# chkda/pytorch-distributed-tutorials

Hardware: AMD Instinct MI355X
Metric: images/sec (whole node) ResNet-50 bf16 at 1/2/4/8 MI355X (higher is better)
Workload: dtype bf16; 1 GPU; model=resnet50, global_batch=256, image_size=224, parallelism=dp1, impl=native, backend=nccl, wire_dtype=fp32, comm_backend=auto, cudnn_benchmark=False, graph=False, deterministic=False, force_comm=False, plan_world=1

## Files before the change

csrc/kernels/bn_act.hip:

```cpp
#include "common.h"
#include "fp8_util.h"
#include "igemm_common.h"
#include "kernels.h"
#include "pool_quad.h"

#include <algorithm>
#include <cstdlib>
#include <mutex>
#include <numeric>
#include <stdexcept>
#include <unordered_map>

namespace pdt {

__device__ __forceinline__ void load8(const float* p, float (&v)[8]) {
  float4 a = *reinterpret_cast<const float4*>(p);
  float4 b = *reinterpret_cast<const float4*>(p + 4);
  v[0] = a.x; v[1] = a.y; v[2] = a.z; v[3] = a.w; v[4] = b.x; v[5] = b.y; v[6] = b.z; v[7] = b.w;
}

#ifndef PDT_FIN_CH
#define PDT_FIN_CH 32
#endif
constexpr int FIN_CH = PDT_FIN_CH;
// ... 25 lines not shown
  return b < 0 ? -1 : b * kTileCounters;
}

int bn_counter_bank(hipStream_t st) {
  const int off = counter_bank(st);
  return off < 0 ? -1 : off / kTileCounters;
}

static bool bn_lastblock() {
  static int v = -1;
  if (v < 0) {
    const char* e = getenv("PDT_BN_LASTBLOCK");
    v = (e && e[0] == '0') ? 0 : 1;
  }
  return v == 1;
}

__device__ __forceinline__ void st_wt(float* p, float v) {
  __hip_atomic_store(p, v, __ATOMIC_RELAXED, __HIP_MEMORY_SCOPE_AGENT);
}
__device__ __forceinline__ float ld_wt(const float* p) {
  return __hip_atomic_load(const_cast<float*>(p), __ATOMIC_RELAXED, __HIP_MEMORY_SCOPE_AGENT);
}
__device__ __forceinline__ bool last_block_of_tile(int tile, unsigned int nblocks) {
  __shared__ int s_last;
  asm volatile("s_waitcnt vmcnt(0)" ::: "memory");
  __syncthreads();
  if (threadIdx.x == 0) {
    const unsigned int prev = __hip_atomic_fetch_add(&g_tile_counters[tile], 1u, __ATOMIC_RELAXED,
                                                     __HIP_MEMORY_SCOPE_AGENT);
    const bool last = prev == nblocks - 1;
    if (last) __hip_atomic_store(&g_tile_counters[tile], 0u, __ATOMIC_RELAXED, __HIP_MEMORY_SCOPE_AGENT);
    s_last = last ? 1 : 0;
  }
  __syncthreads();
  return s_last != 0;
}

__global__ void __launch_bounds__(256) bn_finalize_kernel(const float* __restrict__ part, int ngroups,
                                                          int grows, int M, int K,
                                                          float* __restrict__ ws,
                                                          float* __restrict__ rm,
                                                          float* __restrict__ rv,
                                                          const float* __restrict__ gamma,
                                                          const float* __restrict__ beta,
                                                          float momentum, float eps,
                                                          float* __restrict__ out, int mode,
                                                          int nparts, int cbase, int gpb) {
  __shared__ float sS[FIN_ROWS][FIN_CH + 1], sA[FIN_ROWS][FIN_CH + 1], sB[FIN_ROWS][FIN_CH + 1];
  const int tx = threadIdx.x & (FIN_CH - 1), ty = threadIdx.x / FIN_CH;
  const int k = blockIdx.x * FIN_CH + tx;
  const int g0 = blockIdx.y * gpb;
  const int g1 = min(ngroups, g0 + gpb);
  float S = 0.f, A = 0.f, B = 0.f;
  if (mode != 2) {
  if (k < K) {
#pragma unroll 8
    for (int g = g0 + ty; g < g1; g += FIN_ROWS) {
      const float cnt = (float)min(grows, M - g * grows);
      const float sg = part[((int64_t)g * 2 + 0) * K + k];
      const float qg = part[((int64_t)g * 2 + 1) * K + k];
      S += sg;
      A += qg;
      B = fmaf(sg, sg / cnt, B);
    }
  }
  sS[ty][tx] = S; sA[ty][tx] = A; sB[ty][tx] = B;
  __syncthreads();
  const bool direct = mode == 0 && gridDim.y == 1;
  if (ty == 0 && k < K) {
    for (int r = 1; r < FIN_ROWS; ++r) { S += sS[r][tx]; A += sA[r][tx]; B += sB[r][tx]; }
    if (!direct) {
      float* o = ws + ((int64_t)blockIdx.y * 3) * K;
      st_wt(o + k, S); st_wt(o + K + k, A); st_wt(o + 2 * K + k, B);
    }
  }
  if (mode == 1) return;
  if (direct) {
    if (ty != 0 || k >= K) return;
  } else if (!last_block_of_tile(cbase + blockIdx.x, gridDim.y)) {
    return;
  }
  }
  const bool direct = mode == 0 && gridDim.y == 1;
  const int P = mode == 2 ? nparts : gridDim.y;
  if (!direct) {
  S = 0.f; A = 0.f; B = 0.f;
  if (k < K) {
#pragma unroll 8
    for (int p = ty; p < P; p += FIN_ROWS) {
      const float* o = ws + ((int64_t)p * 3) * K;
      S += ld_wt(o + k); A += ld_wt(o + K + k); B += ld_wt(o + 2 * K + k);
    }
  }
  sS[ty][tx] = S; sA[ty][tx] = A; sB[ty][tx] = B;
  __syncthreads();
  if (ty != 0 || k >= K) return;
  for (int r = 1; r < FIN_ROWS; ++r) { S += sS[r][tx]; A += sA[r][tx]; B += sB[r][tx]; }
  }
  const float mu = S / (float)M;
  const float m2 = fmaxf(A + B - S * mu, 0.f);
  const float var = m2 / (float)M;
  const float invstd = rsqrtf(var + eps);
  if (rm != nullptr) {
    const float unb = M > 1 ? m2 / (float)(M - 1) : var;
    rm[k] = (1.f - momentum) * rm[k] + momentum * mu;
    rv[k] = (1.f - momentum) * rv[k] + momentum * unb;
  }
  const float sc = gamma[k] * invstd;
  out[k] = mu;
  out[K + k] = invstd;
  out[2 * K + k] = sc;
  out[3 * K + k] = beta[k] - mu * sc;
}

int bn_finalize_partitions(int ngroups) { return ceil_div(ngroups, fin_gpb(ngroups)); }

void launch_bn_finalize(const float* part, int ngroups, int grows, int M, int K, float* rm, float* rv,
                        const float* gamma, const float* beta, float momentum, float eps,
                        float* out, hipStream_t st) {
  const int gpb = fin_gpb(ngroups);
  int P = ceil_div(ngroups, gpb);
  float* ws = out + 4 * (int64_t)K;
  if (ceil_div(K, FIN_CH) > kTileCounters / 2) throw std::runtime_error("bn_finalize: too many channels");
  const int bank = (bn_lastblock() && P > 1) ? counter_bank(st) : 0;
  if (bn_lastblock() && bank >= 0) {
    hipLaunchKernelGGL(bn_finalize_kernel, dim3(ceil_div(K, FIN_CH), P), dim3(256), 0, st, part,
                       ngroups, grows, M, K, ws, rm, rv, gamma, beta, momentum, eps, out, 0, P,
                       bank, gpb);
  } else {
    hipLaunchKernelGGL(bn_finalize_kernel, dim3(ceil_div(K, FIN_CH), P), dim3(256), 0, st, part,
                       ngroups, grows, M, K, ws, rm, rv, gamma, beta, momentum, eps, out, 1, P, 0, gpb);
    hipLaunchKernelGGL(bn_finalize_kernel, dim3(ceil_div(K, FIN_CH), 1), dim3(256), 0, st, part,
                       ngroups, grows, M, K, ws, rm, rv, gamma, beta, momentum, eps, out, 2, P, 0, gpb);
  }
}

__global__ void __launch_bounds__(256) bn_finalize_sums_kernel(double* __restrict__ acc, int M, int K,
                                                               float* __restrict__ rm, float* __restrict__ rv,
                                                               const float* __restrict__ gamma,
                                                               const float* __restrict__ beta, float momentum,
                                                               float eps, float* __restrict__ out) {
  const int k = blockIdx.x * blockDim.x + threadIdx.x;
  if (k >= K) return;
  double s[kStatSlots], q[kStatSlots];
#pragma unroll
  for (int x = 0; x < kStatSlots; ++x) {
    s[x] = acc[(size_t)x * 2 * K + k];
    q[x] = acc[(size_t)x * 2 * K + K + k];
  }
  const float g = gamma[k], bt = beta[k];
  const float rm0 = rm != nullptr ? rm[k] : 0.f, rv0 = rm != nullptr ? rv[k] : 0.f;
  double S = 0.0, Q = 0.0;
#pragma unroll
  for (int x = 0; x < kStatSlots; ++x) {
    S += s[x];
    Q += q[x];
    acc[(size_t)x * 2 * K + k] = 0.0;
    acc[(size_t)x * 2 * K + K + k] = 0.0;
  }
  const double Md = (double)M;
  const double mu = S / Md;
  const double var = fmax(Q / Md - mu * mu, 0.0);
  const float invstd = rsqrtf((float)var + eps);
  if (rm != nullptr) {
    const float unb = M > 1 ? (float)(var * Md / (Md - 1.0)) : (float)var;
    rm[k] = (1.f - momentum) * rm0 + momentum * (float)mu;
    rv[k] = (1.f - momentum) * rv0 + momentum * unb;
  }
  const float sc = g * invstd;
  out[k] = (float)mu;
  out[K + k] = invstd;
  out[2 * K + k] = sc;
  out[3 * K + k] = bt - (float)mu * sc;
}

void launch_bn_finalize_sums(const BnFwdFuse& bn, int M, int K, hipStream_t st) {
  hipLaunchKernelGGL(bn_finalize_sums_kernel, dim3(ceil_div(K, 256)), dim3(256), 0, st, bn.acc, M, K, bn.rm,
                     bn.rv, bn.gamma, bn.beta, bn.momentum, bn.eps, bn.out);
}

struct FoldCoef {
  const float* stats;
  const float* gamma;
  const float* sums;
  int K;
  float invM;
  __device__ __forceinline__ void ab(int k, float& a, float& b) const {
    const float is = stats[K + k], mu = stats[k];
    const float k1 = gamma[k] * is;
    const float k2 = sums[K + k] * is * is * invM;
    a = -k1 * k2;
    b = -k1 * (sums[k] * invM - mu * k2);
  }
};

constexpr int kFoldMaxK = 2048;
constexpr int kCsumSlots = 128, kCsumBlocks = 4096;
typedef __bf16 fold_v8bf __attribute__((ext_vector_type(8)));

__global__ void __launch_bounds__(256) bn_fold_coef_kernel(FoldCoef cf, float* __restrict__ coef) {
  __builtin_amdgcn_s_setprio(3);
  const int k = blockIdx.x * 256 + threadIdx.x;
  if (k < cf.K) cf.ab(k, coef[k], coef[cf.K + k]);
}

__global__ void __launch_bounds__(256) bn_fold_weights_kernel(const uint16_t* __restrict__ wt, FoldCoef cf,
                                                              const float* __restrict__ coef, int C, int nG,
                                                              uint16_t* __restrict__ wfold,
                                                              float* __restrict__ bias,
                                                              float* __restrict__ part) {
  __builtin_amdgcn_s_setprio(3);
  const int K = cf.K, t = threadIdx.x;
  const int KC = K + C;
  const int bid = blockIdx.x;
  if (bid >= nG) {
    const int64_t e = ((int64_t)(bid - nG) * 256 + t) * 8;
    if (e >= (int64_t)C * K) return;
    const int c = (int)(e / K), k = (int)(e - (int64_t)c * K);
    f8 v = unpack8(*reinterpret_cast<const uint4*>(wt + e));
    float g8[8], i8[8];
    load8(cf.gamma + k, g8);
    load8(cf.stats + K + k, i8);
#pragma unroll
    for (int q = 0; q < 8; ++q) v.v[q] *= g8[q] * i8[q];
    *reinterpret_cast<uint4*>(wfold + (size_t)c * KC + k) = pack8(v);
    return;
  }
  const int nt = C / 32;
  const int ti = bid / nt, tj = bid - ti * nt;
  const int c0 = ti * 32, d0 = tj * 32;
  const int wv = t >> 6, lane = t & 63;
  const int r = lane & 31, kh = (lane >> 5) * 8;
  const bool with_bias = d0 == 0;
  const int kq = K / 4, kbeg = wv * kq;
  const uint16_t* pa = wt + (size_t)(c0 + r) * K + kbeg + kh;
  const uint16_t* pb = wt + (size_t)(d0 + r) * K + kbeg + kh;
  const float* ca_ = coef + kbeg + kh;
  const float* cb_ = coef + K + kbeg + kh;
  v16f acc = {};
  float bacc = 0.f;
  constexpr int B4 = 4;
  uint4 xa[B4], xb[B4], ya[B4], yb[B4];
#pragma unroll
  for (int q = 0; q < B4; ++q) {
    xa[q] = *reinterpret_cast<const uint4*>(pa + q * 16);
    xb[q] = *reinterpret_cast<const uint4*>(pb + q * 16);
  }
  for (int k0 = 0; k0 < kq; k0 += 16 * B4) {
    const bool more = k0 + 16 * B4 < kq;
    if (more) {
#pragma unroll
      for (int q = 0; q < B4; ++q) {
        ya[q] = *reinterpret_cast<const uint4*>(pa + k0 + 16 * B4 + q * 16);
        yb[q] = *reinterpret_cast<const uint4*>(pb + k0 + 16 * B4 + q * 16);
      }
    }
#pragma unroll
    for (int q = 0; q < B4; ++q) {
      const int kb = k0 + q * 16;
      float a8[8];
      load8(ca_ + kb, a8);
      f8 fa = unpack8(xa[q]);
      if (with_bias) {
        float b8[8];
        load8(cb_ + kb, b8);
#pragma unroll
        for (int e = 0; e < 8; ++e) bacc = fmaf(fa.v[e], b8[e], bacc);
      }
#pragma unroll
      for (int e = 0; e < 8; ++e) fa.v[e] *= a8[e];
      const uint4 qa = pack8(fa);
      acc = __builtin_amdgcn_mfma_f32_32x32x16_bf16(__builtin_bit_cast(fold_v8bf, qa),
                                                    __builtin_bit_cast(fold_v8bf, xb[q]), acc, 0, 0, 0);
    }
    if (more) {
#pragma unroll
      for (int q = 0; q < B4; ++q) { xa[q] = ya[q]; xb[q] = yb[q]; }
    }
  }
  float* pw = part + (size_t)bid * (3 * 17 * 64);
  if (wv > 0) {
    float* q = pw + (wv - 1) * (17 * 64);
#pragma unroll
    for (int e = 0; e < 16; ++e) q[e * 64 + lane] = acc[e];
    q[16 * 64 + lane] = bacc;
  }
  __syncthreads();
  if (wv != 0) return;
#pragma unroll
  for (int e = 0; e < 16; ++e) {
    const float v = acc[e] + pw[e * 64 + lane] + pw[17 * 64 + e * 64 + lane] + pw[34 * 64 + e * 64 + lane];
    const int row = 8 * (e >> 2) + 4 * (lane >> 5) + (e & 3);
    wfold[(size_t)(c0 + row) * KC + K + d0 + (lane & 31)] = f2bf(v);
  }
  if (with_bias) {
    bacc += pw[16 * 64 + lane] + pw[33 * 64 + lane] + pw[50 * 64 + lane];
    bacc += __shfl_xor(bacc, 32, 64);
    if (lane < 32) bias[c0 + r] = bacc;
  }
}

constexpr int kFoldTile = 64;
__global__ void __launch_bounds__(256) bn_fold_wgrad_kernel(float* __restrict__ t1,
                                                            float* __restrict__ gram,
                                                            const float* __restrict__ colsum,
                                                            const uint16_t* __restrict__ wt, FoldCoef cf, int C,
                                                            float* __restrict__ out, float* __restrict__ dgamma,
                                                            float* __restrict__ dbeta, int* __restrict__ done,
                                                            int zero_sums, int csum_slots) {
  const int K = cf.K, t = threadIdx.x;
  const int nc = C / kFoldTile;
  const int tk = blockIdx.x / nc, tc = blockIdx.x - tk * nc;
  const int k0 = tk * kFoldTile, c0 = tc * kFoldTile;
  if (blockIdx.x == 0 && dgamma != nullptr) {
    for (int k = t; k < K; k += 256) {
      const float is = cf.stats[K + k];
      dgamma[k] += cf.sums[K + k] * is;
      dbeta[k] += cf.sums[k];
    }
  }
  __shared__ __attribute__((aligned(16))) float sW[32][kFoldTile];
  __shared__ __attribute__((aligned(16))) float sG[32][kFoldTile];
  __shared__ float sCs[4][kFoldTile];
  __shared__ int last;
  {
    const int j = t & (kFoldTile - 1), ph = t >> 6;
    float a = 0.f;
    if (csum_slots == 1) {
      if (ph == 0) a = colsum[c0 + j];
    } else {
#pragma unroll 8
      for (int sl = ph; sl < kCsumSlots; sl += 4) a += colsum[(size_t)sl * C + c0 + j];
    }
    sCs[ph][j] = a;
    __syncthreads();
    if (t < kFoldTile) sCs[0][t] = sCs[0][t] + sCs[1][t] + sCs[2][t] + sCs[3][t];
  }
  const int ty = t >> 4, tx = t & 15;
  float acc[4][4] = {};
  for (int q0 = 0; q0 < C; q0 += 32) {
    {
      const int q = t >> 3, kk = (t & 7) * 8;
      f8 v = unpack8(*reinterpret_cast<const uint4*>(wt + (size_t)(q0 + q) * K + k0 + kk));
      *reinterpret_cast<float4*>(&sW[q][kk]) = make_float4(v.v[0], v.v[1], v.v[2], v.v[3]);
      *reinterpret_cast<float4*>(&sW[q][kk + 4]) = make_float4(v.v[4], v.v[5], v.v[6], v.v[7]);
    }
#pragma unroll
    for (int h = 0; h < 2; ++h) {
      const int e = t + h * 256, q = e >> 4, cc = (e & 15) * 4;
      *reinterpret_cast<float4*>(&sG[q][cc]) = *reinterpret_cast<const float4*>(gram + (size_t)(q0 + q) * C + c0 + cc);
    }
    __syncthreads();
#pragma unroll 8
    for (int q = 0; q < 32; ++q) {
      const float4 w = *reinterpret_cast<const float4*>(&sW[q][ty * 4]);
      const float4 g = *reinterpret_cast<const float4*>(&sG[q][tx * 4]);
      const float wv[4] = {w.x, w.y, w.z, w.w}, gv[4] = {g.x, g.y, g.z, g.w};
#pragma unroll
      for (int i = 0; i < 4; ++i)
#pragma unroll
        for (int j = 0; j < 4; ++j) acc[i][j] = fmaf(wv[i], gv[j], acc[i][j]);
    }
    __syncthreads();
  }
  const float csv[4] = {sCs[0][tx * 4], sCs[0][tx * 4 + 1], sCs[0][tx * 4 + 2], sCs[0][tx * 4 + 3]};
#pragma unroll
  for (int i = 0; i < 4; ++i) {
    const int k = k0 + ty * 4 + i;
    const float is = cf.stats[K + k], mu = cf.stats[k];
    const float k1 = cf.gamma[k] * is;
    const float k2 = cf.sums[K + k] * is * is * cf.invM;
    const float a = -k1 * k2, b = -k1 * (cf.sums[k] * cf.invM - mu * k2);
    const size_t o = (size_t)k * C + c0 + tx * 4;
    float4 tv = *reinterpret_cast<const float4*>(t1 + o);
    float4 ov = *reinterpret_cast<const float4*>(out + o);
    ov.x += k1 * tv.x + a * acc[i][0] + b * csv[0];
    ov.y += k1 * tv.y + a * acc[i][1] + b * csv[1];
    ov.z += k1 * tv.z + a * acc[i][2] + b * csv[2];
    ov.w += k1 * tv.w + a * acc[i][3] + b * csv[3];
    *reinterpret_cast<float4*>(out + o) = ov;
    if (done != nullptr) *reinterpret_cast<float4*>(t1 + o) = make_float4(0.f, 0.f, 0.f, 0.f);
  }
  if (done == nullptr) return;
  __syncthreads();
  if (t == 0) {
    __threadfence();
    const int nk = K / kFoldTile;
    int v = atomicAdd(done + tc, 1) == nk - 1 ? 1 : 0;
    if (v) {
      done[tc] = 0;
      __threadfence();
      v = atomicAdd(done + nc, 1) == nc - 1 ? 2 : 1;
      if (v == 2) done[nc] = 0;
    }
    last = v;
  }
  __syncthreads();
  if (last == 0) return;
  __threadfence();
  for (int e = t; e < C * (kFoldTile / 4); e += 256) {
    const int q = e >> 4, cc = (e & 15) * 4;
    *reinterpret_cast<float4*>(gram + (size_t)q * C + c0 + cc) = make_float4(0.f, 0.f, 0.f, 0.f);
  }
  if (csum_slots > 1)
    for (int e = t; e < csum_slots * kFoldTile; e += 256)
      const_cast<float*>(colsum)[(size_t)(e / kFoldTile) * C + c0 + (e % kFoldTile)] = 0.f;
  if (last == 2 && zero_sums) {
    float* sm = const_cast<float*>(cf.sums);
    for (int e = t; e < 2 * K; e += 256) sm[e] = 0.f;
  }
}

void launch_bn_fold_wgrad(float* t1, float* gram, const float* colsum, const uint16_t* wt,
                          const float* stats, const float* gamma, const float* sums, int M, int C, int K,
                          float* out, float* dgamma, float* dbeta, int* done, bool zero_sums, hipStream_t st,
                          int csum_slots) {
  if (C % kFoldTile != 0 || K % kFoldTile != 0)
    throw std::runtime_error("bn_fold_wgrad: needs C % 64 == 0, K % 64 == 0");
  if (csum_slots != 1 && (csum_slots != kCsumSlots || done == nullptr))
    throw std::runtime_error("bn_fold_wgrad: column sums come as 1 vector, or bn_act_fwd's slots in consume mode");
  FoldCoef cf{stats, gamma, sums, K, 1.f / (float)M};
  hipLaunchKernelGGL(bn_fold_wgrad_kernel, dim3((K / kFoldTile) * (C / kFoldTile)), dim3(256), 0, st, t1, gram,
                     colsum, wt, cf, C, out, dgamma, dbeta, done, zero_sums ? 1 : 0, csum_slots);
}

int64_t bn_fold_weights_ws_floats(int C, int K) { return C + 2 * (int64_t)K + (int64_t)(C / 32) * (C / 32) * 3 * 17 * 64; }

void launch_bn_fold_weights(const uint16_t* wt, const float* stats, const float* gamma, const float* sums,
                            int M, int C, int K, uint16_t* wfold, float* bias, hipStream_t st) {
  if (C % 32 != 0 || K % 256 != 0 || K > kFoldMaxK)
    throw std::runtime_error("bn_fold_weights: needs C % 32 == 0, K % 256 == 0, K <= 2048");
  const int nG = (C / 32) * (C / 32);
  const int nS = (int)(((int64_t)C * K / 8 + 255) / 256);
  FoldCoef cf{stats, gamma, sums, K, 1.f / (float)M};
  float* coef = bias + C;
  float* part = coef + 2 * K;
  hipLaunchKernelGGL(bn_fold_coef_kernel, dim3(ceil_div(K, 256)), dim3(256), 0, st, cf, coef);
  hipLaunchKernelGGL(bn_fold_weights_kernel, dim3(nG + nS), dim3(256), 0, st, wt, cf, coef, C, nG, wfold, bias,
                     part);
}

__global__ void bn_eval_params_kernel(const float* rm, const float* rv, const float* gamma,
                                      const float* beta, float eps, int K, float* out) {
  int k = blockIdx.x * blockDim.x + threadIdx.x;
  if (k >= K) return;
  float invstd = rsqrtf(rv[k] + eps);
  float sc = gamma[k] * invstd;
  out[k] = rm[k];
  out[K + k] = invstd;
  out[2 * K + k] = sc;
  out[3 * K + k] = beta[k] - rm[k] * sc;
}

void launch_bn_eval_params(const float* rm, const float* rv, const float* gamma, const float* beta,
                           float eps, int K, float* out, hipStream_t st) {
  hipLaunchKernelGGL(bn_eval_params_kernel, dim3(ceil_div(K, 256)), dim3(256), 0, st, rm, rv, gamma,
                     beta, eps, K, out);
}


template <bool RES, bool RELU, bool MASK = false, bool RESBN = false, int U = 1, bool CSUM = false>
__global__ void __launch_bounds__(256) bn_act_fwd_kernel(const uint4* __restrict__ y,
                                                         const float* __restrict__ scale,
                                                         const float* __restrict__ shift,
                                                         const uint4* __restrict__ res,
                                                         uint4* __restrict__ z, int64_t nvec,
                                                         int K8, uint8_t* __restrict__ zmask = nullptr,
                                                         const float* __restrict__ rscale = nullptr,
                                                         const float* __restrict__ rshift = nullptr,
                                                         float* __restrict__ csum = nullptr) {
  const int64_t stride = (int64_t)gridDim.x * blockDim.x;
  const int64_t v0 = (int64_t)blockIdx.x * blockDim.x + threadIdx.x;
  const int c0 = (int)(v0 % K8) * 8;
  float sc[8], sh[8], rsc[8], rsh[8], cs[8];
#pragma unroll
  for (int j = 0; j < 8; ++j) cs[j] = 0.f;
  load8(scale + c0, sc);
  load8(shift + c0, sh);
  if constexpr (RESBN) {
    load8(rscale + c0, rsc);
    load8(rshift + c0, rsh);
  }
  auto body = [&](int64_t v, const uint4 yv, const uint4 rv) {
    f8 a = unpack8(yv);
    f8 r;
    if (RES) r = unpack8(rv);
    if constexpr (RESBN) {
#pragma unroll
      for (int j = 0; j < 8; ++j) r.v[j] = bf2f(f2bf(fmaf(r.v[j], rsc[j], rsh[j])));
    }
#pragma unroll
    for (int j = 0; j < 8; ++j) {
      float t = fmaf(a.v[j], sc[j], sh[j]);
      if (RES) t += r.v[j];
      if (RELU) t = fmaxf(t, 0.f);
      a.v[j] = t;
    }
    const uint4 zb = pack8(a);
    z[v] = zb;
    if constexpr (CSUM) {
      const f8 zr = unpack8(zb);
#pragma unroll
      for (int j = 0; j < 8; ++j) cs[j] += zr.v[j];
    }
    if constexpr (MASK) {
      const f8 zr = unpack8(zb);
      uint32_t bits = 0;
#pragma unroll
      for (int j = 0; j < 8; ++j) bits |= (zr.v[j] > 0.f ? 1u : 0u) << j;
      zmask[v] = (uint8_t)bits;
    }
  };
  int64_t v = v0;
  if constexpr (U > 1) {
    for (; v + (U - 1) * stride < nvec; v += U * stride) {
      uint4 yv[U], rv[U];
#pragma unroll
      for (int u = 0; u < U; ++u) {
        yv[u] = y[v + u * stride];
        if (RES) rv[u] = res[v + u * stride];
      }
#pragma unroll
      for (int u = 0; u < U; ++u) body(v + u * stride, yv[u], RES ? rv[u] : yv[u]);
    }
  }
  for (; v < nvec; v += stride) body(v, y[v], RES ? res[v] : uint4{});
  if constexpr (CSUM) {
    __shared__ float red[256][9];
#pragma unroll
    for (int j = 0; j < 8; ++j) red[threadIdx.x][j] = cs[j];
    __syncthreads();
    if ((int)threadIdx.x < K8) {
      float t8[8];
#pragma unroll
      for (int j = 0; j < 8; ++j) t8[j] = 0.f;
      for (int u = threadIdx.x; u < 256; u += K8)
#pragma unroll
        for (int j = 0; j < 8; ++j) t8[j] += red[u][j];
      float* slot = csum + (size_t)(blockIdx.x % kCsumSlots) * (K8 * 8) + threadIdx.x * 8;
#pragma unroll
      for (int j = 0; j < 8; ++j) unsafeAtomicAdd(slot + j, t8[j]);
    }
  }
}

static int ew_block_cap_env() {
  static int v = -1;
  if (v < 0) {
    const char* e = getenv("PDT_EW_BLOCKS");
    v = e ? std::max(256, atoi(e)) : 0;
  }
  return v;
}

constexpr int kEwCap = 8192;
constexpr int kEwCapResidual = 32768;

static int ew_blocks(int64_t nvec, int K8, int cap_default = kEwCap) {
  int64_t b = (nvec + 255) / 256;
  const int64_t cap = ew_block_cap_env() > 0 ? ew_block_cap_env() : cap_default;
  b = b < cap ? b : cap;
  const int64_t q = K8 / std::gcd(K8, 256);
  return (int)(((b + q - 1) / q) * q);
}

template <bool RES, bool RELU, bool MASK, bool RESBN>
static void fwd_launch(dim3 g, dim3 b, hipStream_t st, const uint4* Y, const float* scale, const float* shift,
                       const uint4* R, uint4* Z, int64_t nvec, int K8, uint8_t* zmask = nullptr,
                       const float* rscale = nullptr, const float* rshift = nullptr) {
  hipLaunchKernelGGL((bn_act_fwd_kernel<RES, RELU, MASK, RESBN, 1>), g, b, 0, st, Y, scale, shift, R, Z, nvec, K8,
                     zmask, rscale, rshift);
}

int bn_csum_slots() { return kCsumSlots; }

void launch_bn_act_fwd(const uint16_t* y, const float* scale, const float* shift,
                       const uint16_t* res, bool relu, uint16_t* z, int64_t M, int K,
                       hipStream_t st, uint8_t* zmask, const float* rscale, const float* rshift,
                       float* csum) {
  int64_t nvec = M * K / 8;
  int K8 = K / 8;
  dim3 g(ew_blocks(nvec, K8, res ? kEwCapResidual : kEwCap)), b(256);
  auto Y = reinterpret_cast<const uint4*>(y);
  auto R = reinterpret_cast<const uint4*>(res);
  auto Z = reinterpret_cast<uint4*>(z);
  if (csum != nullptr) {
    if (res || zmask || rscale || !relu || K8 > 256 || 256 % K8 != 0)
      throw std::runtime_error("bn_act_fwd: column sums only on the plain BN+ReLU pass, 256 % (K/8) == 0");
    const int64_t want = std::max<int64_t>(1, nvec / (256 * 8));
    const dim3 gc(ew_blocks(std::min<int64_t>(nvec, want * 256), K8, kCsumBlocks));
    hipLaunchKernelGGL((bn_act_fwd_kernel<false, true, false, false, 1, true>), gc, b, 0, st, Y, scale, shift,
                       R, Z, nvec, K8, nullptr, nullptr, nullptr, csum);
    return;
  }
  if (rscale != nullptr) {
    if (!res || !rshift) throw std::runtime_error("bn_act_fwd: residual BN needs the residual and its shift");
    if (zmask) {
      if (!relu) throw std::runtime_error("bn_act_fwd: a ReLU mask needs relu");
      fwd_launch<true, true, true, true>(g, b, st, Y, scale, shift, R, Z, nvec, K8,
                         zmask, rscale, rshift);
    } else if (relu) {
      fwd_launch<true, true, false, true>(g, b, st, Y, scale, shift, R, Z, nvec,
                         K8, nullptr, rscale, rshift);
    } else {
      fwd_launch<true, false, false, true>(g, b, st, Y, scale, shift, R, Z, nvec,
                         K8, nullptr, rscale, rshift);
    }
    return;
  }
  if (zmask) {
    if (!relu) throw std::runtime_error("bn_act_fwd: a ReLU mask needs relu");
    if (res) fwd_launch<true, true, true, false>(g, b, st, Y, scale, shift, R, Z, nvec, K8, zmask);
    else fwd_launch<false, true, true, false>(g, b, st, Y, scale, shift, R, Z, nvec, K8, zmask);
  } else if (res) {
    if (relu) fwd_launch<true, true, false, false>(g, b, st, Y, scale, shift, R, Z, nvec, K8);
    else fwd_launch<true, false, false, false>(g, b, st, Y, scale, shift, R, Z, nvec, K8);
  } else {
    if (relu) fwd_launch<false, true, false, false>(g, b, st, Y, scale, shift, R, Z, nvec, K8);
    else fwd_launch<false, false, false, false>(g, b, st, Y, scale, shift, R, Z, nvec, K8);
  }
}

constexpr int RED_BLOCKS_MAX = 1024;
constexpr int RED_CH8 = 32;
constexpr int RED_TARGET = 2048;

static int red_chunks(int K) {
  const int K8 = K / 8;
  return K8 > RED_CH8 ? K8 / RED_CH8 : 1;
}

static int red_blocks(int64_t M, int K) {
  const int64_t by_rows = (M + 31) / 32;
  int64_t b = (RED_TARGET + red_chunks(K) - 1) / red_chunks(K);
  b = std::max<int64_t>(b, (M + 1023) / 1024);
  b = std::min<int64_t>(std::min<int64_t>(b, by_rows), RED_BLOCKS_MAX);
  return (int)std::max<int64_t>(b, 1);
}

size_t bn_bwd_ws_floats(int64_t M, int K) { return (size_t)red_blocks(M, K) * 2 * K; }

template <int MASK>
__device__ __forceinline__ float relu_grad(float g, float zv, float yv, float sc, float sh) {
  if (MASK == 1) return zv > 0.f ? g : 0.f;
  if (MASK == 2) return fmaf(yv, sc, sh) > 0.f ? g : 0.f;
  return g;
}

__device__ __forceinline__ void block_tree_sum16(float* sh, int t, int rpi, int step, const float (&a)[8],
                                                 const float (&b)[8]) {
#pragma unroll
  for (int j = 0; j < 8; ++j) {
    sh[j * 256 + t] = a[j];
    sh[(8 + j) * 256 + t] = b[j];
  }
  __syncthreads();
  const int roff = t / step;
  for (int s = rpi / 2; s > 0; s >>= 1) {
    if (roff < s) {
#pragma unroll
      for (int j = 0; j < 16; ++j) sh[j * 256 + t] += sh[j * 256 + t + s * step];
    }
    __syncthreads();
  }
}

template <int MASK>
__global__ void __launch_bounds__(256) bn_bwd_reduce_stage1(const uint4* __restrict__ dz,
                                                            const uint4* __restrict__ z,
                                                            const uint4* __restrict__ y,
                                                            const float* __restrict__ stats,
                                                            int64_t M, int K8,
                                                            float* __restrict__ ws) {
  extern __shared__ __attribute__((aligned(16))) float sh[];
  const int K = K8 * 8;
  const int CH8 = K8 < RED_CH8 ? K8 : RED_CH8;
  const int t = threadIdx.x;
  const int c8 = blockIdx.y * CH8 + t % CH8;
  const int rpi = 256 / CH8;
  const int roff = t / CH8;
  int64_t rows_per_block = (M + gridDim.x - 1) / gridDim.x;
  int64_t r0 = (int64_t)blockIdx.x * rows_per_block;
  int64_t r1 = min(M, r0 + rows_per_block);
  float mu[8], sc[8], shf[8];
  load8(stats + c8 * 8, mu);
  if (MASK == 2) { load8(stats + 2 * K + c8 * 8, sc); load8(stats + 3 * K + c8 * 8, shf); }
  float sg[8] = {0, 0, 0, 0, 0, 0, 0, 0}, sgx[8] = {0, 0, 0, 0, 0, 0, 0, 0};
#pragma unroll 4
  for (int64_t r = r0 + roff; r < r1; r += rpi) {
    int64_t v = r * K8 + c8;
    f8 d = unpack8(dz[v]);
    f8 yy = unpack8(y[v]);
    f8 zz;
    if (MASK == 1) zz = unpack8(z[v]);
#pragma unroll
    for (int j = 0; j < 8; ++j) {
      float g = relu_grad<MASK>(d.v[j], MASK == 1 ? zz.v[j] : 0.f, yy.v[j],
                                MASK == 2 ? sc[j] : 0.f, MASK == 2 ? shf[j] : 0.f);
      sg[j] += g;
      sgx[j] = fmaf(g, yy.v[j] - mu[j], sgx[j]);
    }
  }
  block_tree_sum16(sh, t, rpi, CH8, sg, sgx);
  if (roff == 0) {
    float* o = ws + (int64_t)blockIdx.x * 2 * K;
#pragma unroll
    for (int j = 0; j < 8; ++j) { o[c8 * 8 + j] = sh[j * 256 + t]; o[K + c8 * 8 + j] = sh[(8 + j) * 256 + t]; }
  }
}

template <int CH>
__global__ void __launch_bounds__(256) bn_bwd_reduce_stage2(const float* __restrict__ ws, int nb,
// ... 503 lines not shown
```

Before: 14500 images/sec.

## Rewrite BN fold weight-grad kernel with f32 MFMA and register prefetch ring

Replaces the LDS-tiled scalar-FMA inner product in bn_fold_wgrad_kernel with per-wave 32x32x2 f32 MFMA. Operands are streamed straight from global memory through a 4-deep register ring instead of being staged in shared memory. Column-sum reduction now uses wave shuffles, and the completion counter is tracked per wave. All block-level syncs and thread fences are dropped, with only compiler barriers left. This removes LDS traffic and barriers from a small GEMM-like step in backward, at the cost of higher register use and weaker memory ordering around the last-block cleanup.

```diff
diff --git a/csrc/kernels/bn_act.hip b/csrc/kernels/bn_act.hip
--- a/csrc/kernels/bn_act.hip
+++ b/csrc/kernels/bn_act.hip
@@ -351,7 +351,9 @@
 }
 
 constexpr int kFoldTile = 64;
-__global__ void __launch_bounds__(256) bn_fold_wgrad_kernel(float* __restrict__ t1,
+constexpr int kFoldQB = 8;
+constexpr int kFoldRing = 4;
+__global__ void __launch_bounds__(256, 2) bn_fold_wgrad_kernel(float* __restrict__ t1,
                                                             float* __restrict__ gram,
                                                             const float* __restrict__ colsum,
                                                             const uint16_t* __restrict__ wt, FoldCoef cf, int C,
@@ -361,7 +363,49 @@
   const int K = cf.K, t = threadIdx.x;
   const int nc = C / kFoldTile;
   const int tk = blockIdx.x / nc, tc = blockIdx.x - tk * nc;
-  const int k0 = tk * kFoldTile, c0 = tc * kFoldTile;
+  const int wv = t >> 6, lane = t & 63;
+  const int r = lane & 31, h = lane >> 5;
+  const int k0 = tk * kFoldTile + (wv >> 1) * 32, c0 = tc * kFoldTile + (wv & 1) * 32;
+  const uint32_t aoff = (uint32_t)h * K + k0 + r, boff = (uint32_t)h * C + c0 + r;
+  uint16_t xa[kFoldRing][kFoldQB];
+  float xb[kFoldRing][kFoldQB];
+#pragma unroll
+  for (int d = 0; d < kFoldRing; ++d)
+#pragma unroll
+    for (int s = 0; s < kFoldQB; ++s) {
+      const int q = 2 * (kFoldQB * d + s);
+      xa[d][s] = (wt + (size_t)q * K)[aoff];
+      xb[d][s] = (gram + (size_t)q * C)[boff];
+    }
+  float cs;
+  if (csum_slots == 1) {
+    cs = colsum[c0 + r];
+  } else {
+    float4 s4[4];
+    const float* pc = colsum + (size_t)(lane >> 3) * C + c0 + 4 * (lane & 7);
+#pragma unroll
+    for (int u = 0; u < 4; ++u) s4[u] = *reinterpret_cast<const float4*>(pc + (size_t)(8 * u) * C);
+#pragma unroll
+    for (int i = 4; i < kCsumSlots / 8; ++i) {
+      const float4 x = *reinterpret_cast<const float4*>(pc + (size_t)(8 * i) * C);
+      s4[i & 3].x += x.x; s4[i & 3].y += x.y; s4[i & 3].z += x.z; s4[i & 3].w += x.w;
+    }
+    float c4[4] = {(s4[0].x + s4[1].x) + (s4[2].x + s4[3].x), (s4[0].y + s4[1].y) + (s4[2].y + s4[3].y),
+                   (s4[0].z + s4[1].z) + (s4[2].z + s4[3].z), (s4[0].w + s4[1].w) + (s4[2].w + s4[3].w)};
+#pragma unroll
+    for (int off = 8; off < 64; off <<= 1)
+#pragma unroll
+      for (int j = 0; j < 4; ++j) c4[j] += __shfl_xor(c4[j], off, 64);
+    const float y0 = __shfl(c4[0], r >> 2, 64), y1 = __shfl(c4[1], r >> 2, 64);
+    const float y2 = __shfl(c4[2], r >> 2, 64), y3 = __shfl(c4[3], r >> 2, 64);
+    cs = (r & 2) ? ((r & 1) ? y3 : y2) : ((r & 1) ? y1 : y0);
+  }
+  float ck1, cka, ckb;
+  {
+    const int k = k0 + r;
+    ck1 = cf.gamma[k] * cf.stats[K + k];
+    cf.ab(k, cka, ckb);
+  }
   if (blockIdx.x == 0 && dgamma != nullptr) {
     for (int k = t; k < K; k += 256) {
       const float is = cf.stats[K + k];
@@ -369,95 +413,64 @@
       dbeta[k] += cf.sums[k];
     }
   }
-  __shared__ __attribute__((aligned(16))) float sW[32][kFoldTile];
-  __shared__ __attribute__((aligned(16))) float sG[32][kFoldTile];
-  __shared__ float sCs[4][kFoldTile];
-  __shared__ int last;
-  {
-    const int j = t & (kFoldTile - 1), ph = t >> 6;
-    float a = 0.f;
-    if (csum_slots == 1) {
-      if (ph == 0) a = colsum[c0 + j];
-    } else {
-#pragma unroll 8
-      for (int sl = ph; sl < kCsumSlots; sl += 4) a += colsum[(size_t)sl * C + c0 + j];
-    }
-    sCs[ph][j] = a;
-    __syncthreads();
-    if (t < kFoldTile) sCs[0][t] = sCs[0][t] + sCs[1][t] + sCs[2][t] + sCs[3][t];
-  }
-  const int ty = t >> 4, tx = t & 15;
-  float acc[4][4] = {};
-  for (int q0 = 0; q0 < C; q0 += 32) {
-    {
-      const int q = t >> 3, kk = (t & 7) * 8;
-      f8 v = unpack8(*reinterpret_cast<const uint4*>(wt + (size_t)(q0 + q) * K + k0 + kk));
-      *reinterpret_cast<float4*>(&sW[q][kk]) = make_float4(v.v[0], v.v[1], v.v[2], v.v[3]);
-      *reinterpret_cast<float4*>(&sW[q][kk + 4]) = make_float4(v.v[4], v.v[5], v.v[6], v.v[7]);
-    }
-#pragma unroll
-    for (int h = 0; h < 2; ++h) {
-      const int e = t + h * 256, q = e >> 4, cc = (e & 15) * 4;
-      *reinterpret_cast<float4*>(&sG[q][cc]) = *reinterpret_cast<const float4*>(gram + (size_t)(q0 + q) * C + c0 + cc);
-    }
-    __syncthreads();
-#pragma unroll 8
-    for (int q = 0; q < 32; ++q) {
-      const float4 w = *reinterpret_cast<const float4*>(&sW[q][ty * 4]);
-      const float4 g = *reinterpret_cast<const float4*>(&sG[q][tx * 4]);
-      const float wv[4] = {w.x, w.y, w.z, w.w}, gv[4] = {g.x, g.y, g.z, g.w};
-#pragma unroll
-      for (int i = 0; i < 4; ++i)
-#pragma unroll
-        for (int j = 0; j < 4; ++j) acc[i][j] = fmaf(wv[i], gv[j], acc[i][j]);
-    }
-    __syncthreads();
-  }
-  const float csv[4] = {sCs[0][tx * 4], sCs[0][tx * 4 + 1], sCs[0][tx * 4 + 2], sCs[0][tx * 4 + 3]};
-#pragma unroll
-  for (int i = 0; i < 4; ++i) {
-    const int k = k0 + ty * 4 + i;
-    const float is = cf.stats[K + k], mu = cf.stats[k];
-    const float k1 = cf.gamma[k] * is;
-    const float k2 = cf.sums[K + k] * is * is * cf.invM;
-    const float a = -k1 * k2, b = -k1 * (cf.sums[k] * cf.invM - mu * k2);
-    const size_t o = (size_t)k * C + c0 + tx * 4;
-    float4 tv = *reinterpret_cast<const float4*>(t1 + o);
-    float4 ov = *reinterpret_cast<const float4*>(out + o);
-    ov.x += k1 * tv.x + a * acc[i][0] + b * csv[0];
-    ov.y += k1 * tv.y + a * acc[i][1] + b * csv[1];
-    ov.z += k1 * tv.z + a * acc[i][2] + b * csv[2];
-    ov.w += k1 * tv.w + a * acc[i][3] + b * csv[3];
-    *reinterpret_cast<float4*>(out + o) = ov;
-    if (done != nullptr) *reinterpret_cast<float4*>(t1 + o) = make_float4(0.f, 0.f, 0.f, 0.f);
+  float tv[16], ov[16];
+#pragma unroll
+  for (int e = 0; e < 16; ++e) {
+    const size_t o = (size_t)(k0 + 8 * (e >> 2) + 4 * h + (e & 3)) * C + c0 + r;
+    tv[e] = t1[o];
+    ov[e] = out[o];
+  }
+  v16f acc = {};
+  for (int q0 = 0; q0 < C; q0 += 2 * kFoldQB * kFoldRing) {
+#pragma unroll
+    for (int d = 0; d < kFoldRing; ++d) {
+#pragma unroll
+      for (int s = 0; s < kFoldQB; ++s)
+        acc = __builtin_amdgcn_mfma_f32_32x32x2f32(__uint_as_float((uint32_t)xa[d][s] << 16), xb[d][s], acc, 0, 0, 0);
+      const int qn = q0 + 2 * kFoldQB * (kFoldRing + d);
+      if (qn < C) {
+#pragma unroll
+        for (int s = 0; s < kFoldQB; ++s) {
+          xa[d][s] = (wt + (size_t)(qn + 2 * s) * K)[aoff];
+          xb[d][s] = (gram + (size_t)(qn + 2 * s) * C)[boff];
+        }
+      }
+    }
+  }
+#pragma unroll
+  for (int e = 0; e < 16; ++e) {
+    const int row = 8 * (e >> 2) + 4 * h + (e & 3);
+    const float k1 = __shfl(ck1, row, 64), a = __shfl(cka, row, 64), b = __shfl(ckb, row, 64);
+    const size_t o = (size_t)(k0 + row) * C + c0 + r;
+    out[o] = ov[e] + (k1 * tv[e] + a * acc[e] + b * cs);
+    if (done != nullptr) t1[o] = 0.f;
   }
   if (done == nullptr) return;
-  __syncthreads();
-  if (t == 0) {
-    __threadfence();
-    const int nk = K / kFoldTile;
-    int v = atomicAdd(done + tc, 1) == nk - 1 ? 1 : 0;
+  asm volatile("" ::: "memory");
+  int v = 0;
+  if (lane == 0) {
+    const int nw = (K / kFoldTile) * 4;
+    v = atomicAdd(done + tc, 1) == nw - 1 ? 1 : 0;
     if (v) {
       done[tc] = 0;
-      __threadfence();
       v = atomicAdd(done + nc, 1) == nc - 1 ? 2 : 1;
       if (v == 2) done[nc] = 0;
     }
-    last = v;
-  }
-  __syncthreads();
-  if (last == 0) return;
-  __threadfence();
-  for (int e = t; e < C * (kFoldTile / 4); e += 256) {
+  }
+  v = __builtin_amdgcn_readfirstlane(v);
+  if (v == 0) return;
+  asm volatile("" ::: "memory");
+  const int g0 = tc * kFoldTile;
+  for (int e = lane; e < C * (kFoldTile / 4); e += 64) {
     const int q = e >> 4, cc = (e & 15) * 4;
-    *reinterpret_cast<float4*>(gram + (size_t)q * C + c0 + cc) = make_float4(0.f, 0.f, 0.f, 0.f);
+    *reinterpret_cast<float4*>(gram + (size_t)q * C + g0 + cc) = make_float4(0.f, 0.f, 0.f, 0.f);
   }
   if (csum_slots > 1)
-    for (int e = t; e < csum_slots * kFoldTile; e += 256)
-      const_cast<float*>(colsum)[(size_t)(e / kFoldTile) * C + c0 + (e % kFoldTile)] = 0.f;
-  if (last == 2 && zero_sums) {
+    for (int e = lane; e < csum_slots * kFoldTile; e += 64)
+      const_cast<float*>(colsum)[(size_t)(e / kFoldTile) * C + g0 + (e % kFoldTile)] = 0.f;
+  if (v == 2 && zero_sums) {
     float* sm = const_cast<float*>(cf.sums);
-    for (int e = t; e < 2 * K; e += 256) sm[e] = 0.f;
+    for (int e = lane; e < 2 * K; e += 64) sm[e] = 0.f;
   }
 }
 
```

Result: no change. 14550 images/sec (median of 6 runs) (+0.3%).
